# henriChevreux/distillation_trajectories

Hardware: AMD Instinct MI355X
Metric: trajectory-timesteps/sec (B×T U-Net fwd) at 16×16 T=50 (higher is better)
Workload: dtype f32 (fp32-accurate; convolutions: exact 3-plane bf16 operand split on bf16 MFMA with fp32 accumulate, or native fp32 MFMA, chosen per layer)

## Files before the change

### distillation_trajectories_amd/csrc/dt_conv_strip.hip

```cpp
#include <mutex>
#include <type_traits>

#include "dt_conv_epilogue.h"

namespace dt {

extern __shared__ __attribute__((aligned(16))) __bf16 strip_lds[];

template <int BM, int BN, int KC, int WK>
__global__ __launch_bounds__(256, find_strip_form(BM, BN, KC, WK)->waves_per_simd()) void conv_strip_bf16x6_kernel(const ConvParams p) {
  constexpr ConvForm F = *find_strip_form(BM, BN, KC, WK);
  constexpr int WN = F.wn(), WM = F.wm(), NT = 256;
  constexpr int MI = F.mi(), NI = F.ni();
  constexpr int KW = F.kw();
  static_assert(WM * WN * WK * 64 == NT && KC % WK == 0 && MI * 32 * WM == BM && NI * 32 * WN == BN && (WK == 1 || (MI == 2 && NI == 2)), "wave layout");
  constexpr int PLANE_B = F.plane_b(), STAGE_B = 3 * PLANE_B;
  constexpr int AP = F.ap();
  static_assert(2 * (BM + 2 * (F.max_w() + 1)) <= AP * NT, "strip staging reach");
  const int halo = strip_halo(p.W, BM);
  const int R = F.strip_rows(halo);
  const int RZ = F.zero_row(R);
  const int PLANE_A = F.plane_a(RZ);
  __bf16 *As = strip_lds;
  __bf16 *Bs = strip_lds + F.strip_elems(PLANE_A);

  const int tid = threadIdx.x, lane = tid & 63;
  const int wave = __builtin_amdgcn_readfirstlane(tid >> 6);
  const int wk = wave % WK, wm = (wave / WK) / WN, wn = (wave / WK) % WN;
  const int half = lane >> 5, l31 = lane & 31;
  const int m0 = blockIdx.x * BM, n0 = blockIdx.y * BN;
  const int HW = p.H * p.W;
  const int CC = p.cin_p >> 4;

  bool s_in[AP], s_ok[AP], s_core[AP];
  int s_off[AP], s_off2[AP], s_offb[AP], s_lds[AP];
#pragma unroll
  for (int i = 0; i < AP; ++i) {
    const int item = tid + i * NT;
    const int srow = item >> 1, hh = item & 1;
    const int m = m0 - halo + srow;
    s_in[i] = item < 2 * R;
    s_ok[i] = s_in[i] && m >= 0 && m < p.M;
    s_core[i] = s_ok[i] && srow >= halo && srow < halo + BM;
    const int mm = s_ok[i] ? m : 0;
    s_off[i] = mm * p.cin_p + hh * 8;
    s_off2[i] = mm * p.cin2_p + hh * 8;
    s_offb[i] = mm * p.b_stride + hh * 8;
    s_lds[i] = srow * 16 + ((hh ^ ((srow >> 3) & 1)) << 3);
  }
  constexpr bool B_ALL = WK > 1 && BN * 4 == NT;
  constexpr int NB = B_ALL ? KC * 3 / 2 : KC * 3, SB = B_ALL ? 2 : 1;
  static_assert(!B_ALL || (KC * 3) % 2 == 0, "weight staging");
  const bool b_thread = B_ALL || tid < BN * 2;
  const int bt = B_ALL ? (tid & (BN * 2 - 1)) : tid, bsub = B_ALL ? tid / (BN * 2) : 0;
  const size_t w_plane = (size_t)p.n_p * 16;
  const __bf16 *wbase = reinterpret_cast<const __bf16 *>(p.w) + (size_t)n0 * 16 + bt * 8 + bsub * w_plane;
  const __bf16 *wbase2 = reinterpret_cast<const __bf16 *>(p.w2) + (size_t)n0 * 16 + bt * 8 + bsub * w_plane;
  const int b_lds = bsub * PLANE_B + bt * 8;

  int a_row[MI];
  unsigned a_mask[MI];
#pragma unroll
  for (int mi = 0; mi < MI; ++mi) {
    const int row_i = wm * (MI * 32) + mi * 32 + l31;
    const int m = m0 + row_i;
    a_row[mi] = row_i + halo;
    unsigned mask = 0;
    if (m < p.M) {
      const int rem = m % HW;
      const int y = rem / p.W, x = rem - y * p.W;
#pragma unroll
      for (int t = 0; t < 9; ++t) {
        const int yy = y + t / 3 - 1, xx = x + t % 3 - 1;
        if (yy >= 0 && yy < p.H && xx >= 0 && xx < p.W) mask |= 1u << t;
      }
    }
    a_mask[mi] = mask;
  }
  int b_frag[NI];
#pragma unroll
  for (int ni = 0; ni < NI; ++ni) {
    const int row = wn * (NI * 32) + ni * 32 + l31;
    b_frag[ni] = row * 16 + ((half ^ ((row >> 3) & 1)) << 3);
  }

  f32x16 acc[MI][NI];
#pragma unroll
  for (int mi = 0; mi < MI; ++mi)
#pragma unroll
    for (int ni = 0; ni < NI; ++ni)
#pragma unroll
      for (int r = 0; r < 16; ++r) acc[mi][ni][r] = 0.f;

  const int n_main = (CC + p.splits * KC - 1) / (p.splits * KC);
  const int cc0 = blockIdx.z * n_main * KC;
  const int CC2 = p.cin2_p >> 4;
  const int n_chunks = n_main + (p.in2 ? (CC2 + KC - 1) / KC : 0);

  f32x4 sa0[KC][AP], sa1[KC][AP];
  u32x4 rb[NB];
  auto load_strip = [&](int ch) __attribute__((always_inline)) {
#pragma unroll
    for (int kk = 0; kk < KC; ++kk)
#pragma unroll
    for (int i = 0; i < AP; ++i) {
      sa0[kk][i] = f32x4{0.f, 0.f, 0.f, 0.f}; sa1[kk][i] = sa0[kk][i];
      if (ch < n_main) {
        const int cc = cc0 + ch * KC + kk;
        if (s_ok[i] && cc < CC) {
          const float *src = (p.in_b && cc >= p.cc_a) ? p.in_b + s_offb[i] + (cc - p.cc_a) * 16 : p.in + s_off[i] + cc * 16;
          sa0[kk][i] = *reinterpret_cast<const f32x4 *>(src);
          sa1[kk][i] = *reinterpret_cast<const f32x4 *>(src + 4);
        }
      } else if (s_core[i] && (ch - n_main) * KC + kk < CC2) {
        const int c2 = (ch - n_main) * KC + kk;
        const float *src = (p.in2_b && c2 >= p.cc_a) ? p.in2_b + s_offb[i] + (c2 - p.cc_a) * 16 : p.in2 + s_off2[i] + c2 * 16;
        sa0[kk][i] = *reinterpret_cast<const f32x4 *>(src);
        sa1[kk][i] = *reinterpret_cast<const f32x4 *>(src + 4);
      }
    }
  };
  auto write_strip = [&]() __attribute__((always_inline)) {
#pragma unroll
    for (int kk = 0; kk < KC; ++kk)
#pragma unroll
    for (int i = 0; i < AP; ++i)
      if (s_in[i]) {
        bf16x8 p1, p2, p3;
        split8(sa0[kk][i], sa1[kk][i], p1, p2, p3);
        __bf16 *A = As + kk * 3 * PLANE_A;
        *reinterpret_cast<bf16x8 *>(A + s_lds[i]) = p1;
        *reinterpret_cast<bf16x8 *>(A + PLANE_A + s_lds[i]) = p2;
        *reinterpret_cast<bf16x8 *>(A + 2 * PLANE_A + s_lds[i]) = p3;
      }
  };
  const size_t tap_stride = (size_t)p.ccw * 3 * w_plane, group_stride = (size_t)KC * 3 * w_plane;
  const __bf16 *wrun = wbase + (size_t)cc0 * 3 * w_plane;
  enum { ADV_NONE = 0, ADV_TAP, ADV_GROUP, ADV_SKIP0, ADV_SKIP };
  auto load_b = [&](int adv) __attribute__((always_inline)) {
    if (adv == ADV_TAP) wrun += tap_stride;
    else if (adv == ADV_GROUP) wrun = wrun - 8 * tap_stride + group_stride;
    else if (adv == ADV_SKIP0) wrun = wbase2;
    else if (adv == ADV_SKIP) wrun += group_stride;
    if (b_thread) {
#pragma unroll
      for (int i = 0; i < NB; ++i)
        rb[i] = *reinterpret_cast<const u32x4 *>(wrun + (SB * i) * w_plane);
    }
  };
  auto write_b = [&](int stage) __attribute__((always_inline)) {
    if (b_thread) {
      __bf16 *B = Bs + stage * KC * STAGE_B;
#pragma unroll
      for (int i = 0; i < NB; ++i) *reinterpret_cast<u32x4 *>(B + (SB * i) * PLANE_B + b_lds) = rb[i];
    }
  };

  constexpr bool DB = WK > 1;
  bf16x8 fbn[KW][NI][3];
  auto load_bd = [&](int adv) __attribute__((always_inline)) {
    if (adv == ADV_TAP) wrun += tap_stride;
    else if (adv == ADV_GROUP) wrun = wrun - 8 * tap_stride + group_stride;
    else if (adv == ADV_SKIP0) wrun = wbase2;
    else if (adv == ADV_SKIP) wrun += group_stride;
    const __bf16 *wt = wrun - (bt * 8 + bsub * w_plane);
#pragma unroll
    for (int kw = 0; kw < KW; ++kw)
#pragma unroll
      for (int ni = 0; ni < NI; ++ni)
#pragma unroll
        for (int pl = 0; pl < 3; ++pl)
          fbn[kw][ni][pl] = *reinterpret_cast<const bf16x8 *>(wt + ((wk * KW + kw) * 3 + pl) * w_plane + b_frag[ni]);
  };

  load_strip(0);
  if (DB) load_bd(ADV_NONE); else load_b(ADV_NONE);
  if (tid < 48 * KC) *reinterpret_cast<u32x4 *>(As + (tid >> 4) * PLANE_A + RZ * 16 + (tid & 15) * 8) = u32x4{0u, 0u, 0u, 0u};
  write_strip();
  if (!DB) write_b(0);
  __syncthreads();

  int step = 0;
  bool stage_next_strip = true;
  auto do_step = [&](auto TT, int ch, bool first_tap, bool last_tap, bool next_chunk, int adv) __attribute__((always_inline)) {
    constexpr int tt = decltype(TT)::value;
    const bool more = !last_tap || next_chunk;
    if (first_tap && next_chunk && stage_next_strip) load_strip(ch + 1);
    bf16x8 fbc[KW][NI][3];
    if (DB) {
#pragma unroll
      for (int kw = 0; kw < KW; ++kw)
#pragma unroll
        for (int ni = 0; ni < NI; ++ni)
#pragma unroll
          for (int pl = 0; pl < 3; ++pl) fbc[kw][ni][pl] = fbn[kw][ni][pl];
      if (more) load_bd(adv);
    } else if (more) load_b(adv);
    {
      int wv = p.W;
      asm volatile("" : "+s"(wv));
      const int shift = (tt / 3 - 1) * wv + (tt % 3 - 1);
      int a_e[MI];
#pragma unroll
      for (int mi = 0; mi < MI; ++mi) {
        int row0 = a_row[mi];
        asm volatile("" : "+v"(row0));
        const int srow = row0 + shift;
        const int lrow = ((a_mask[mi] >> tt) & 1u) ? srow : RZ + (srow & 7);
        a_e[mi] = lrow * 16 + ((half ^ ((srow >> 3) & 1)) << 3);
      }
#pragma unroll
      for (int kw = 0; kw < KW; ++kw) {
        const int kk = wk * KW + kw;
        const __bf16 *A = As + kk * 3 * PLANE_A;
        const __bf16 *B = Bs + ((step & 1) * KC + kk) * STAGE_B;
        bf16x8 fb[NI][3];
#pragma unroll
        for (int ni = 0; ni < NI; ++ni)
#pragma unroll
          for (int pl = 0; pl < 3; ++pl)
            fb[ni][pl] = DB ? fbc[kw][ni][pl] : *reinterpret_cast<const bf16x8 *>(B + pl * PLANE_B + b_frag[ni]);
#pragma unroll
        for (int mi = 0; mi < MI; ++mi) {
          bf16x8 fa[3];
#pragma unroll
          for (int pl = 0; pl < 3; ++pl)
            fa[pl] = *reinterpret_cast<const bf16x8 *>(A + pl * PLANE_A + a_e[mi]);
#pragma unroll
          for (int ni = 0; ni < NI; ++ni) mfma_bf16x6(acc[mi][ni], fa, fb[ni]);
        }
      }
    }
    if (!DB && more) write_b((step + 1) & 1);
    const bool restage = last_tap && next_chunk && stage_next_strip;
    if (restage) {
      __syncthreads();
      write_strip();
    }
    if (!DB || restage) __syncthreads();
    ++step;
  };

  constexpr bool DIRECT = MI * KW <= 2 && KC >= 2;
  f32x4 ga0[KW][MI][2], ga1[KW][MI][2];
  const int n_skip = p.in2 ? (CC2 + KC - 1) / KC : 0;
  auto load_a = [&](f32x4 (&g)[KW][MI][2], int s2) __attribute__((always_inline)) {
#pragma unroll
    for (int kw = 0; kw < KW; ++kw)
#pragma unroll
      for (int mi = 0; mi < MI; ++mi) {
        const int c2 = s2 * KC + wk * KW + kw;
        const int m = m0 + wm * (MI * 32) + mi * 32 + l31;
        g[kw][mi][0] = f32x4{0.f, 0.f, 0.f, 0.f}; g[kw][mi][1] = g[kw][mi][0];
        if (m < p.M && c2 < CC2) {
          const float *src = (p.in2_b && c2 >= p.cc_a) ? p.in2_b + (size_t)m * p.b_stride + (c2 - p.cc_a) * 16 + half * 8
                                                       : p.in2 + (size_t)m * p.cin2_p + c2 * 16 + half * 8;
          g[kw][mi][0] = *reinterpret_cast<const f32x4 *>(src);
          g[kw][mi][1] = *reinterpret_cast<const f32x4 *>(src + 4);
        }
      }
  };
  auto skip_step = [&](f32x4 (&g)[KW][MI][2], int s2) __attribute__((always_inline)) {
    const bool more = s2 + 1 < n_skip;
    bf16x8 fbc[KW][NI][3];
    if (DB) {
#pragma unroll
      for (int kw = 0; kw < KW; ++kw)
#pragma unroll
        for (int ni = 0; ni < NI; ++ni)
#pragma unroll
          for (int pl = 0; pl < 3; ++pl) fbc[kw][ni][pl] = fbn[kw][ni][pl];
      if (more) load_bd(ADV_SKIP);
    } else if (more) load_b(ADV_SKIP);
#pragma unroll
    for (int kw = 0; kw < KW; ++kw) {
      const int kk = wk * KW + kw;
      const __bf16 *B = Bs + ((step & 1) * KC + kk) * STAGE_B;
      bf16x8 fb[NI][3];
#pragma unroll
      for (int ni = 0; ni < NI; ++ni)
#pragma unroll
        for (int pl = 0; pl < 3; ++pl) fb[ni][pl] = DB ? fbc[kw][ni][pl] : *reinterpret_cast<const bf16x8 *>(B + pl * PLANE_B + b_frag[ni]);
#pragma unroll
      for (int mi = 0; mi < MI; ++mi) {
        bf16x8 fa[3];
        split8(g[kw][mi][0], g[kw][mi][1], fa[0], fa[1], fa[2]);
#pragma unroll
        for (int ni = 0; ni < NI; ++ni) mfma_bf16x6(acc[mi][ni], fa, fb[ni]);
      }
    }
    if (s2 + 2 < n_skip) load_a(g, s2 + 2);
    if (!DB) {
      if (more) write_b((step + 1) & 1);
      __syncthreads();
    }
    ++step;
  };

  const int prio_grp = ((blockIdx.x + gridDim.x * (blockIdx.y + gridDim.y * blockIdx.z)) >> 8) & 1;
  const bool use_prio = gridDim.x * gridDim.y * gridDim.z <= 512;
  for (int ch = 0; ch < n_main; ++ch) {
    if (use_prio) {
      if ((ch ^ prio_grp) & 1) __builtin_amdgcn_s_setprio(1);
      else __builtin_amdgcn_s_setprio(0);
    }
    const bool next_chunk = ch + 1 < ((WK > 1 && p.in2) ? n_main : n_chunks);
    if (DIRECT && WK == 1 && p.in2 && ch + 1 == n_main) {
      stage_next_strip = false;
      load_a(ga0, 0);
      if (n_skip > 1) load_a(ga1, 1);
    }
    do_step(std::integral_constant<int, 0>{}, ch, true, false, next_chunk, ADV_TAP);
    do_step(std::integral_constant<int, 1>{}, ch, false, false, next_chunk, ADV_TAP);
    do_step(std::integral_constant<int, 2>{}, ch, false, false, next_chunk, ADV_TAP);
    do_step(std::integral_constant<int, 3>{}, ch, false, false, next_chunk, ADV_TAP);
    do_step(std::integral_constant<int, 4>{}, ch, false, false, next_chunk, ADV_TAP);
    do_step(std::integral_constant<int, 5>{}, ch, false, false, next_chunk, ADV_TAP);
    do_step(std::integral_constant<int, 6>{}, ch, false, false, next_chunk, ADV_TAP);
    do_step(std::integral_constant<int, 7>{}, ch, false, false, next_chunk, ADV_TAP);
    do_step(std::integral_constant<int, 8>{}, ch, false, true, next_chunk, ch + 1 < n_main ? ADV_GROUP : ADV_SKIP0);
    if constexpr (WK == 1) {
      if (ch + 1 == n_main && p.in2) conv_midpoint<MI, NI>(p, acc, n0, wn, l31);
    }
  }
  if constexpr (WK > 1) {
    if (p.in2) {
      constexpr int P = F.pitch(), COPY = F.copy_floats();
      float *red = reinterpret_cast<float *>(strip_lds);
#pragma unroll
      for (int mi = 0; mi < MI; ++mi) {
        if (mi || DB) __syncthreads();
#pragma unroll
        for (int ni = 0; ni < NI; ++ni)
#pragma unroll
          for (int r = 0; r < 16; ++r)
            red[wk * COPY + (wm * 32 + 4 * half + (r & 3) + 8 * (r >> 2)) * P + wn * (NI * 32) + ni * 32 + l31] = acc[mi][ni][r];
        __syncthreads();
#pragma unroll
        for (int ni = 0; ni < NI; ++ni)
#pragma unroll
          for (int r = 0; r < 16; ++r) {
            const float *src = red + (wm * 32 + 4 * half + (r & 3) + 8 * (r >> 2)) * P + wn * (NI * 32) + ni * 32 + l31;
            float v = src[0];
#pragma unroll
            for (int c = 1; c < WK; ++c) v += src[c * COPY];
            acc[mi][ni][r] = wk == 0 ? v : 0.f;
          }
      }
      if (wk == 0) conv_midpoint<MI, NI>(p, acc, n0, wn, l31);
      __syncthreads();
      if (DB) load_bd(ADV_SKIP0); else load_b(ADV_SKIP0);
      if (DIRECT) {
        load_a(ga0, 0);
        if (n_skip > 1) load_a(ga1, 1);
      } else {
        load_strip(n_main);
        if (tid < 48 * KC) *reinterpret_cast<u32x4 *>(As + (tid >> 4) * PLANE_A + RZ * 16 + (tid & 15) * 8) = u32x4{0u, 0u, 0u, 0u};
        write_strip();
      }
      if (!DB) write_b(step & 1);
      __syncthreads();
    }
  }
  __builtin_amdgcn_s_setprio(0);
  if (DIRECT) {
    for (int s2 = 0; s2 < n_skip; s2 += 2) {
      skip_step(ga0, s2);
      if (s2 + 1 < n_skip) skip_step(ga1, s2 + 1);
    }
  } else {
    for (int ch = n_main; ch < n_chunks; ++ch)
      do_step(std::integral_constant<int, 4>{}, ch, true, true, ch + 1 < n_chunks, ADV_SKIP);
  }
  conv_epilogue<BM, BN, WK>(p, acc, reinterpret_cast<float *>(strip_lds), m0, n0, wm, wn, half, l31, wk);
}

#define DT_STRIP_ROW(cls, kind, bm, bn, kc, wk) {{kind, bm, bn, kc, wk, cls}, conv_strip_bf16x6_kernel<bm, bn, kc, wk>},
static const ConvKernel kStripKernels[] = {DT_CONV_FORMS_ALL_STRIP(DT_STRIP_ROW)};

static int strip_lds_attribute() {
  constexpr int kMaxDevices = 64;
  static std::mutex mu;
  static int status[kMaxDevices];
  int dev = 0;
  DT_HIP_TRY(hipGetDevice(&dev));
  if (dev < 0 || dev >= kMaxDevices) return DT_E_ARG;
  std::lock_guard<std::mutex> lock(mu);
  if (status[dev] == 0) {
    status[dev] = 1;
    for (const ConvKernel &k : kStripKernels) {
      if (!k.form.needs_lds_attribute()) continue;
      const hipError_t e = hipFuncSetAttribute(reinterpret_cast<const void *>(k.fn), hipFuncAttributeMaxDynamicSharedMemorySize, (int)k.form.lds_limit());
      if (e != hipSuccess) status[dev] = -(int)e;
    }
  }
  return status[dev] == 1 ? DT_OK : -status[dev];
}

int launch_conv_strip(const ConvParams &p_in, hipStream_t s) {
  ConvParams p = p_in;
  const ConvKernel &k = conv_kernel_of(kStripKernels, p);
  size_t lds = k.form.lds_bytes(p.W);
  p.dup_stage2 = p.n_dup == 2 && p.pool_out && k.form.dup_stage_bytes() <= k.form.lds_limit();
  if (p.dup_stage2 && k.form.dup_stage_bytes() > lds) lds = k.form.dup_stage_bytes();
  if (const int st = k.form.needs_lds_attribute() ? strip_lds_attribute() : DT_OK) return st;
  k.fn<<<dim3((p.M + p.bm - 1) / p.bm, p.n_p / p.bn, p.splits), 256, lds, s>>>(p);
  DT_LAUNCH_CHECK();
  return DT_OK;
}

}
```

Before: 354,600.

## Make strip loads unconditional, prefetch A fragments one MFMA group ahead, move B writes mid-step

Strip loads no longer branch per element. Each channel chunk computes one base pointer and stride, always loads, and zeroes out-of-range or dead rows with a bitmask when writing to LDS. In the register-double-buffered weight path, A-operand LDS fragments are now read one MFMA group ahead (including the next tap's first fragment), with sched_group_barrier hints to interleave LDS reads with MFMAs. For WK==1, KC==2, the B-stage LDS write moves into the middle of the kw loop. These changes aim to hide LDS latency and cut divergent branches, at the cost of extra registers and loads from clamped addresses.

Result: slower. 344,800 (-2.8%).

```diff
diff --git a/distillation_trajectories_amd/csrc/dt_conv_strip.hip b/distillation_trajectories_amd/csrc/dt_conv_strip.hip
--- a/distillation_trajectories_amd/csrc/dt_conv_strip.hip
+++ b/distillation_trajectories_amd/csrc/dt_conv_strip.hip
@@ -33,7 +33,8 @@
   const int CC = p.cin_p >> 4;
 
   bool s_in[AP], s_ok[AP], s_core[AP];
-  int s_off[AP], s_off2[AP], s_offb[AP], s_lds[AP];
+  int s_m[AP], s_lds[AP];
+  const int s_hh8 = (tid & 1) * 8;
 #pragma unroll
   for (int i = 0; i < AP; ++i) {
     const int item = tid + i * NT;
@@ -42,10 +43,7 @@
     s_in[i] = item < 2 * R;
     s_ok[i] = s_in[i] && m >= 0 && m < p.M;
     s_core[i] = s_ok[i] && srow >= halo && srow < halo + BM;
-    const int mm = s_ok[i] ? m : 0;
-    s_off[i] = mm * p.cin_p + hh * 8;
-    s_off2[i] = mm * p.cin2_p + hh * 8;
-    s_offb[i] = mm * p.b_stride + hh * 8;
+    s_m[i] = s_ok[i] ? m : 0;
     s_lds[i] = srow * 16 + ((hh ^ ((srow >> 3) & 1)) << 3);
   }
   constexpr bool B_ALL = WK > 1 && BN * 4 == NT;
@@ -99,40 +97,52 @@
 
   f32x4 sa0[KC][AP], sa1[KC][AP];
   u32x4 rb[NB];
+  auto pick = [](bool c, auto a, auto b) __attribute__((always_inline)) { return c ? a : b; };
+  auto strip_source = [&](int ch, int kk, const float *&base, int &stride) __attribute__((always_inline)) {
+    const bool main = ch < n_main;
+    const int c = main ? cc0 + ch * KC + kk : (ch - n_main) * KC + kk;
+    const float *src_a = pick(main, p.in, p.in2), *src_b = pick(main, p.in_b, p.in2_b);
+    const bool live = c < pick(main, CC, CC2);
+    const bool second = live && src_b && c >= p.cc_a;
+    base = second ? src_b + (c - p.cc_a) * 16 : src_a + (live ? c * 16 : 0);
+    stride = pick(second, p.b_stride, pick(main, p.cin_p, p.cin2_p));
+    return live;
+  };
   auto load_strip = [&](int ch) __attribute__((always_inline)) {
 #pragma unroll
-    for (int kk = 0; kk < KC; ++kk)
-#pragma unroll
-    for (int i = 0; i < AP; ++i) {
-      sa0[kk][i] = f32x4{0.f, 0.f, 0.f, 0.f}; sa1[kk][i] = sa0[kk][i];
-      if (ch < n_main) {
-        const int cc = cc0 + ch * KC + kk;
-        if (s_ok[i] && cc < CC) {
-          const float *src = (p.in_b && cc >= p.cc_a) ? p.in_b + s_offb[i] + (cc - p.cc_a) * 16 : p.in + s_off[i] + cc * 16;
-          sa0[kk][i] = *reinterpret_cast<const f32x4 *>(src);
-          sa1[kk][i] = *reinterpret_cast<const f32x4 *>(src + 4);
-        }
-      } else if (s_core[i] && (ch - n_main) * KC + kk < CC2) {
-        const int c2 = (ch - n_main) * KC + kk;
-        const float *src = (p.in2_b && c2 >= p.cc_a) ? p.in2_b + s_offb[i] + (c2 - p.cc_a) * 16 : p.in2 + s_off2[i] + c2 * 16;
+    for (int kk = 0; kk < KC; ++kk) {
+      const float *base;
+      int stride;
+      strip_source(ch, kk, base, stride);
+#pragma unroll
+      for (int i = 0; i < AP; ++i) {
+        const float *src = base + s_hh8 + s_m[i] * stride;
         sa0[kk][i] = *reinterpret_cast<const f32x4 *>(src);
         sa1[kk][i] = *reinterpret_cast<const f32x4 *>(src + 4);
       }
     }
   };
-  auto write_strip = [&]() __attribute__((always_inline)) {
-#pragma unroll
-    for (int kk = 0; kk < KC; ++kk)
-#pragma unroll
-    for (int i = 0; i < AP; ++i)
-      if (s_in[i]) {
-        bf16x8 p1, p2, p3;
-        split8(sa0[kk][i], sa1[kk][i], p1, p2, p3);
-        __bf16 *A = As + kk * 3 * PLANE_A;
-        *reinterpret_cast<bf16x8 *>(A + s_lds[i]) = p1;
-        *reinterpret_cast<bf16x8 *>(A + PLANE_A + s_lds[i]) = p2;
-        *reinterpret_cast<bf16x8 *>(A + 2 * PLANE_A + s_lds[i]) = p3;
-      }
+  auto write_strip = [&](int ch) __attribute__((always_inline)) {
+    const bool main = ch < n_main;
+#pragma unroll
+    for (int kk = 0; kk < KC; ++kk) {
+      const float *base;
+      int stride;
+      const bool live = strip_source(ch, kk, base, stride);
+#pragma unroll
+      for (int i = 0; i < AP; ++i)
+        if (s_in[i]) {
+          const unsigned keep = live && pick(main, s_ok[i], s_core[i]) ? ~0u : 0u;
+          const f32x4 v0 = __builtin_bit_cast(f32x4, __builtin_bit_cast(u32x4, sa0[kk][i]) & keep);
+          const f32x4 v1 = __builtin_bit_cast(f32x4, __builtin_bit_cast(u32x4, sa1[kk][i]) & keep);
+          bf16x8 p1, p2, p3;
+          split8(v0, v1, p1, p2, p3);
+          __bf16 *A = As + kk * 3 * PLANE_A;
+          *reinterpret_cast<bf16x8 *>(A + s_lds[i]) = p1;
+          *reinterpret_cast<bf16x8 *>(A + PLANE_A + s_lds[i]) = p2;
+          *reinterpret_cast<bf16x8 *>(A + 2 * PLANE_A + s_lds[i]) = p3;
+        }
+    }
   };
   const size_t tap_stride = (size_t)p.ccw * 3 * w_plane, group_stride = (size_t)KC * 3 * w_plane;
   const __bf16 *wrun = wbase + (size_t)cc0 * 3 * w_plane;
@@ -176,12 +186,31 @@
   load_strip(0);
   if (DB) load_bd(ADV_NONE); else load_b(ADV_NONE);
   if (tid < 48 * KC) *reinterpret_cast<u32x4 *>(As + (tid >> 4) * PLANE_A + RZ * 16 + (tid & 15) * 8) = u32x4{0u, 0u, 0u, 0u};
-  write_strip();
+  write_strip(0);
   if (!DB) write_b(0);
   __syncthreads();
 
   int step = 0;
   bool stage_next_strip = true;
+  auto a_elem = [&](auto TT, int mi) __attribute__((always_inline)) {
+    constexpr int tt = decltype(TT)::value;
+    int wv = p.W;
+    asm volatile("" : "+s"(wv));
+    const int shift = (tt / 3 - 1) * wv + (tt % 3 - 1);
+    int row0 = a_row[mi];
+    asm volatile("" : "+v"(row0));
+    const int srow = row0 + shift;
+    const int lrow = ((a_mask[mi] >> tt) & 1u) ? srow : RZ + (srow & 7);
+    return lrow * 16 + ((half ^ ((srow >> 3) & 1)) << 3);
+  };
+  auto read_a = [&](bf16x8 (&fa)[3], int kk, int a_e) __attribute__((always_inline)) {
+    const __bf16 *A = As + kk * 3 * PLANE_A;
+#pragma unroll
+    for (int pl = 0; pl < 3; ++pl) fa[pl] = *reinterpret_cast<const bf16x8 *>(A + pl * PLANE_A + a_e);
+  };
+  constexpr bool PRE_A = false;
+  constexpr bool B_MID = WK == 1 && KC == 2;
+  bf16x8 fa_pre[3];
   auto do_step = [&](auto TT, int ch, bool first_tap, bool last_tap, bool next_chunk, int adv) __attribute__((always_inline)) {
     constexpr int tt = decltype(TT)::value;
     const bool more = !last_tap || next_chunk;
@@ -197,23 +226,18 @@
       if (more) load_bd(adv);
     } else if (more) load_b(adv);
     {
-      int wv = p.W;
-      asm volatile("" : "+s"(wv));
-      const int shift = (tt / 3 - 1) * wv + (tt % 3 - 1);
       int a_e[MI];
 #pragma unroll
-      for (int mi = 0; mi < MI; ++mi) {
-        int row0 = a_row[mi];
-        asm volatile("" : "+v"(row0));
-        const int srow = row0 + shift;
-        const int lrow = ((a_mask[mi] >> tt) & 1u) ? srow : RZ + (srow & 7);
-        a_e[mi] = lrow * 16 + ((half ^ ((srow >> 3) & 1)) << 3);
+      for (int mi = 0; mi < MI; ++mi) a_e[mi] = a_elem(TT, mi);
+      if (DB && first_tap) {
+        read_a(fa_pre, wk * KW, a_e[0]);
+        __builtin_amdgcn_sched_group_barrier(0x100, 3, 0);
       }
 #pragma unroll
       for (int kw = 0; kw < KW; ++kw) {
         const int kk = wk * KW + kw;
-        const __bf16 *A = As + kk * 3 * PLANE_A;
         const __bf16 *B = Bs + ((step & 1) * KC + kk) * STAGE_B;
+        if (B_MID && !first_tap && kw == 1 && more) write_b((step + 1) & 1);
         bf16x8 fb[NI][3];
 #pragma unroll
         for (int ni = 0; ni < NI; ++ni)
@@ -223,19 +247,34 @@
 #pragma unroll
         for (int mi = 0; mi < MI; ++mi) {
           bf16x8 fa[3];
-#pragma unroll
-          for (int pl = 0; pl < 3; ++pl)
-            fa[pl] = *reinterpret_cast<const bf16x8 *>(A + pl * PLANE_A + a_e[mi]);
+          if (DB) {
+#pragma unroll
+            for (int pl = 0; pl < 3; ++pl) fa[pl] = fa_pre[pl];
+            constexpr int TN = tt < 8 ? tt + 1 : tt;
+            const int nb = kw * MI + mi + 1;
+            if (nb < KW * MI) read_a(fa_pre, wk * KW + nb / MI, a_e[nb % MI]);
+            else if (!last_tap) read_a(fa_pre, wk * KW, a_elem(std::integral_constant<int, TN>{}, 0));
+          } else if (PRE_A && kw == 0 && mi == 0 && !first_tap) {
+#pragma unroll
+            for (int pl = 0; pl < 3; ++pl) fa[pl] = fa_pre[pl];
+          } else {
+            read_a(fa, kk, a_e[mi]);
+          }
 #pragma unroll
           for (int ni = 0; ni < NI; ++ni) mfma_bf16x6(acc[mi][ni], fa, fb[ni]);
+          if (DB) {
+            if (kw * MI + mi + 1 < KW * MI || !last_tap) __builtin_amdgcn_sched_group_barrier(0x100, 3, 0);
+            __builtin_amdgcn_sched_group_barrier(0x008, NI * 6, 0);
+          }
         }
       }
     }
-    if (!DB && more) write_b((step + 1) & 1);
+    if (PRE_A && !last_tap) read_a(fa_pre, 0, a_elem(std::integral_constant<int, (tt < 8 ? tt + 1 : tt)>{}, 0));
+    if (!DB && (!B_MID || first_tap) && more) write_b((step + 1) & 1);
     const bool restage = last_tap && next_chunk && stage_next_strip;
     if (restage) {
       __syncthreads();
-      write_strip();
+      write_strip(ch + 1);
     }
     if (!DB || restage) __syncthreads();
     ++step;
@@ -356,7 +395,7 @@
       } else {
         load_strip(n_main);
         if (tid < 48 * KC) *reinterpret_cast<u32x4 *>(As + (tid >> 4) * PLANE_A + RZ * 16 + (tid & 15) * 8) = u32x4{0u, 0u, 0u, 0u};
-        write_strip();
+        write_strip(n_main);
       }
       if (!DB) write_b(step & 1);
       __syncthreads();
```
